# mlakolar/CoordinateDescent.jl

Measured on AMD Instinct MI355X. Metric: coord_updates_per_sec, higher is better.
Workload: dtype f64; 1 GPU; lasso_full_cyclic_sweep_gaussian_n10000000_p1000_f64_allmove; n=10000000, p=1000, s=100, sweep_mode=block32, graph=False, parallelism=rows1

## Files before the change

### coordinatedescent.jl_amd/csrc/cdhip.hip

```cpp
#include "../../include/cdhip.h"

#include <dlfcn.h>
#include <hip/hip_runtime.h>

#include <algorithm>
#include <cmath>
#include <cstdio>
#include <cstdlib>
#include <cstring>
#include <string>
#include <utility>
#include <vector>

#include "kernels.hpp"
#include "gram_kernels.hpp"
#include "vc_kernels.hpp"
#include "vc_gram.hpp"
#include "p2p_exchange.hpp"
#include "sparse_iterate.hpp"
#include "resid_state.hpp"
#include "cache_state.hpp"
#include "exchange_state.hpp"

using namespace cdk;
// ... 281 lines not shown
    int mode = CDH_SWEEP_BLOCK, blockB = 32;
    bool width_default = true, width_agreed = false;
    bool use_graph = false;
    int screening = 1;
    bool reuse_residual = false;
    cdh::ResidState rs;
    bool chunk_dup = false;
    std::vector<int32_t> stamp;
    GraphCache graphs;
    bool graph_broken = false;
    bool domain_error = false;
    int step_grid = 1, block_grid = 1, cus = 1;
    int64_t gram_units = 1;
    Knobs knobs;
    cdh::ExchangeState xs;
    DevBuf<unsigned long long> p2p_inbox;
    cdk::P2PPeers p2p_peers{};
    std::vector<void*> p2p_mapped;
    PinBuf<int> p2p_timeout;
    DevBuf<unsigned> d_p2p_base;
    PinBuf<double> h_xchg;
    size_t h_xchg_doubles = 0;
    GradCache gc;
    CovSolvePath cs;
    SmallPath small;
    bool prof = false;
    double prof_ms = 0.0, prof_bytes = 0.0;
    int64_t prof_launches = 0;
    hipEvent_t ev0 = nullptr, ev1 = nullptr;
    std::string err;
};

#include "quad_solve_types.hpp"
static_assert(kQuadMaxP == CDH_QUAD_MAX_P, "cdhip.h names the limit quad_solve_types.hpp derives");
struct cdh_quad_s {
    int64_t p = 0, max_batch = 0, m = 0;
    int32_t device = 0;
    hipStream_t stream = nullptr;
    unsigned lds_bytes = 0;
    bool A_set = false, penalty_set = false, has_omega = false, omega_shared = false;
    DevBuf<double> A, inv_a, B, omega, lambda0, grid, beta, g, h_out;
    DevBuf<int32_t> sup, nnz, list;
    int64_t list_cap = 0;
    DevBuf<QuadStat> stats;
    PinBuf<QuadStat> h_stats;
    PinBuf<double> h_h;
    std::vector<double> h_B, h_omega, h_lambda0, h_beta;
    std::vector<int32_t> h_sup, h_nnz;
    bool host_stale = true;
};

namespace {

#define HIPCHK(h, call)                                                                     \
    do {                                                                                    \
        hipError_t e_ = (call);                                                             \
        if (e_ != hipSuccess) {                                                             \
            char buf_[512];                                                                 \
            snprintf(buf_, sizeof buf_, "%s failed: %s (%s:%d)", #call, hipGetErrorString(e_), \
                     __FILE__, __LINE__);                                                   \
            (h)->err = buf_;                                                                \
            return e_ == hipErrorOutOfMemory ? CDH_OOM : CDH_HIP_ERROR;                     \
        }                                                                                   \
    } while (0)

#define CHK(call)                                   \
    do {                                            \
        int32_t s_ = (call);                        \
        if (s_ != CDH_OK) return s_;                \
    } while (0)

int32_t fail(cdh_handle h, int32_t code, const char* msg) {
    if (h) h->err = msg; else g_create_error = msg;
    return code;
}

#define NEED_P(h, ptr)                                                         \
    do {                                                                       \
        if (!(ptr)) return fail((h), CDH_BAD_ARG, #ptr " is NULL");            \
    } while (0)

inline int64_t round_up(int64_t a, int64_t b) { return (a + b - 1) / b * b; }

inline int balanced_grid(int64_t units, int64_t gmax) {
    return (int)std::max<int64_t>(1, std::min<int64_t>(gmax, units));
}

template <typename F> int32_t dispatch(cdh_handle h, F&& f) {
    return h->dtype == CDH_F64 ? f((double*)nullptr) : f((float*)nullptr);
}

int32_t upload_ctrl(cdh_handle h) {
    *h->h_ctrl = h->ctrl;
    HIPCHK(h, hipMemcpyAsync(h->d_ctrl, h->h_ctrl, sizeof(Ctrl), hipMemcpyHostToDevice, h->stream));
    return CDH_OK;
}

inline int32_t refused(cdh_handle h, const cdh::Refusal& r) { return r.status == CDH_OK ? (int32_t)CDH_OK : fail(h, r.status, r.msg); }
int32_t exchange_alive(cdh_handle h) { return refused(h, h->xs.alive()); }
int32_t p2p_check(cdh_handle h) {
    if (h->xs.direct_on() && *(volatile int*)h->p2p_timeout) return refused(h, h->xs.p2p_timed_out());
    return CDH_OK;
}

static_assert(GramRec<4>::N <= cdk::kP2PMaxCount, "the widest block record must fit one inbox slot");
cdk::P2PCall next_p2p_call(cdh_handle h) {
    cdh::ExchangeState& xs = h->xs;
    return cdk::P2PCall{h->p2p_peers, xs.rank(), xs.direct_ranks(), xs.next_epoch(), h->knobs.p2p_spin_limit, h->p2p_timeout,
                        xs.in_capture() ? (const unsigned*)h->d_p2p_base : nullptr};
}

int32_t allreduce(cdh_handle h, double* dbuf, size_t count) {
    cdh::ExchangeState& xs = h->xs;
    const cdh::Routing to = xs.route(count);
    switch (to.route) {
    case cdh::Route::Refuse: return refused(h, to.why);
    case cdh::Route::Nothing: return CDH_OK;
    case cdh::Route::Host:
        for (size_t o = 0; o < count; o += h->h_xchg_doubles) {
            const size_t cnt = std::min(h->h_xchg_doubles, count - o);
            HIPCHK(h, hipMemcpyAsync(h->h_xchg, dbuf + o, sizeof(double) * cnt, hipMemcpyDeviceToHost, h->stream));
            HIPCHK(h, hipStreamSynchronize(h->stream));
            const int32_t rc = xs.host_callback()(xs.host_context(), h->h_xchg, (int64_t)cnt);
            if (rc != 0) return fail(h, CDH_RCCL_ERROR, "the host exchange callback reported a failure");
            HIPCHK(h, hipMemcpyAsync(dbuf + o, h->h_xchg, sizeof(double) * cnt, hipMemcpyHostToDevice, h->stream));
            HIPCHK(h, hipStreamSynchronize(h->stream));
        }
        break;
    case cdh::Route::Direct:
        CHK(p2p_check(h));
        for (size_t o = 0; o < count; o += cdk::kP2PMaxCount) {
            const int c = (int)std::min<size_t>(cdk::kP2PMaxCount, count - o);
            hipLaunchKernelGGL(cdk::k_p2p_allreduce, dim3((c + 255) / 256), dim3(256), 0, h->stream, dbuf + o, c,
                               next_p2p_call(h));
            xs.issued(to.route);
        }
        HIPCHK(h, hipGetLastError());
        return CDH_OK;
    case cdh::Route::Rccl: {
        const int rc = g_rccl.AllReduce(dbuf, dbuf, count, kNcclDouble, kNcclSum, xs.communicator(), h->stream);
        if (rc != 0) {
            h->err = std::string("ncclAllReduce failed: ") +
                     (g_rccl.GetErrorString ? g_rccl.GetErrorString(rc) : "?");
            return CDH_RCCL_ERROR;
        }
        break;
    }
    }
    xs.issued(to.route);
    return CDH_OK;
}

int32_t rebuild_residual_from(cdh_handle h, const cdh::SupportList& x, bool with_beta);
int32_t sync_r(cdh_handle h) {
    cdh::ResidState& rs = h->rs;
    if (rs.lazy()) return rebuild_residual_from(h, rs.take_lazy(), false);
    if (rs.pending().empty()) return CDH_OK;
    rs.catchup_begins();
    const cdh::MoveLedger& L = rs.pending();
    for (size_t o = 0; o < L.size(); o += 64) {
        const int cnt = (int)std::min<size_t>(64, L.size() - o);
        for (int i = 0; i < cnt; ++i) { h->h_idx[i] = L[o + (size_t)i]; h->h_hs[i] = L.value(L[o + (size_t)i]); }
        HIPCHK(h, hipMemcpyAsync(h->d_idx, h->h_idx, sizeof(int64_t) * (size_t)cnt, hipMemcpyHostToDevice, h->stream));
        HIPCHK(h, hipMemcpyAsync(h->d_hs, h->h_hs, sizeof(double) * (size_t)cnt, hipMemcpyHostToDevice, h->stream));
        CHK(dispatch(h, [&](auto* t) {
            using T = std::remove_pointer_t<decltype(t)>;
            hipLaunchKernelGGL(k_multi_axpy<T>, dim3(h->step_grid), dim3(kBlock), 0, h->stream, (const T*)h->X, h->ld,
                               h->nvec, (T*)h->r, h->d_idx, h->d_hs, 0, cnt);
            return CDH_OK;
        }));
        HIPCHK(h, hipGetLastError());
        HIPCHK(h, hipStreamSynchronize(h->stream));
        rs.catchup_batch_applied();
    }
    rs.catchup_done();
    h->gc.n_reconcile += 1;
    return CDH_OK;
}

constexpr int64_t kColBatch = 4096;
inline int col_dots_chunks(const cdh_handle_s* h, int64_t bc) {
    const int64_t groups = (bc + kColGroup - 1) / kColGroup;
    const int64_t want_chunks = std::max<int64_t>(1, ((int64_t)h->cus * 8 + groups - 1) / groups);
    return (int)std::max<int64_t>(1, std::min<int64_t>({(int64_t)kColChunks, want_chunks, (h->nvec + kBlock - 1) / kBlock}));
}
int32_t col_dots(cdh_handle h, int64_t j0, int64_t nc, const void* rvec, bool use_w,
                 const int64_t* d_cols = nullptr) {
    if (rvec == h->r) CHK(sync_r(h));
    for (int64_t b0 = 0; b0 < nc; b0 += kColBatch) {
        const int64_t bc = std::min<int64_t>(kColBatch, nc - b0);
        const int64_t groups = (bc + kColGroup - 1) / kColGroup;
        const int chunks = col_dots_chunks(h, bc);
        if ((size_t)groups * chunks * 2 * kColGroup > h->partials_doubles) return fail(h, CDH_BAD_ARG, "partials too small");
        dim3 grid(chunks, (unsigned)groups);
        CHK(dispatch(h, [&](auto* t) {
            using T = std::remove_pointer_t<decltype(t)>;
            hipLaunchKernelGGL(k_col_dots<T>, grid, dim3(kBlock), 0, h->stream, (const T*)h->X, h->ld,
                               h->nvec, use_w ? (const T*)h->w : (const T*)nullptr, (const T*)rvec,
                               j0 + b0, (int)bc, d_cols, h->d_partials);
            return CDH_OK;
        }));
        hipLaunchKernelGGL(k_col_dots_reduce, dim3((unsigned)bc), dim3(64), 0, h->stream,
                           h->d_partials, chunks, h->d_colout + 2 * b0);
        HIPCHK(h, hipGetLastError());
    }
    CHK(allreduce(h, h->d_colout, (size_t)(2 * nc)));
    return CDH_OK;
}

int32_t col_loadings(cdh_handle h) {
    CHK(sync_r(h));
    for (int64_t b0 = 0; b0 < h->p; b0 += kColBatch) {
        const int64_t bc = std::min<int64_t>(kColBatch, h->p - b0);
        const int64_t groups = (bc + kColGroup - 1) / kColGroup;
        const int chunks = col_dots_chunks(h, bc);
        if ((size_t)groups * chunks * kColGroup > h->partials_doubles) return fail(h, CDH_BAD_ARG, "partials too small");
        dim3 grid(chunks, (unsigned)groups);
        CHK(dispatch(h, [&](auto* t) {
            using T = std::remove_pointer_t<decltype(t)>;
            hipLaunchKernelGGL(k_col_loadings<T>, grid, dim3(kBlock), 0, h->stream, (const T*)h->X, h->ld,
                               h->nvec, (const T*)h->r, b0, (int)bc, h->d_partials);
            return CDH_OK;
        }));
        hipLaunchKernelGGL(k_col_loadings_reduce, dim3((unsigned)bc), dim3(64), 0, h->stream,
                           h->d_partials, chunks, h->d_colout + b0);
        HIPCHK(h, hipGetLastError());
    }
    CHK(allreduce(h, h->d_colout, (size_t)h->p));
    return CDH_OK;
}

int32_t resid_moments_dev(cdh_handle h, const void* vec = nullptr, double shift = 0.0, bool sum_w = false) {
    if (!vec) { CHK(sync_r(h)); vec = h->r; }
    const int grid = (int)std::max<int64_t>(1, std::min<int64_t>(1024, (h->nvec + kBlock - 1) / kBlock));
    CHK(dispatch(h, [&](auto* t) {
        using T = std::remove_pointer_t<decltype(t)>;
        auto go = [&](auto kernel) {
            hipLaunchKernelGGL(kernel, dim3(grid), dim3(kBlock), 0, h->stream, h->nvec,
                               (const T*)vec, h->has_w ? (const T*)h->w : (const T*)nullptr, h->d_partials, shift, h->n);
        };
        if (sum_w) go(k_resid_moments<T, true>); else go(k_resid_moments<T>);
        return CDH_OK;
    }));
    hipLaunchKernelGGL(k_sum_records, dim3(1), dim3(kBlock), 0, h->stream, h->d_partials, grid, h->d_red);
    HIPCHK(h, hipGetLastError());
    CHK(allreduce(h, h->d_red, 4));
    return CDH_OK;
}

constexpr int kGcEngage = 3;
constexpr int kGcBusy = 64;
constexpr int kGcMaxFetch = 64;
constexpr int kGcMaxSupport = 512;
constexpr size_t kGcMaxBytes = (size_t)1 << 30;
constexpr int64_t kGcCovWindow = 2048;
constexpr int64_t kGcRowsPerNnz = 400;
constexpr int64_t kGcRowsPerNnzDev = 32;
inline int64_t gc_rows_per_nnz(const cdh_handle_s* h) {
    const GradCache& c = h->gc;
    if (h->knobs.gc_rows_per_nnz > 0) return h->knobs.gc_rows_per_nnz;
    return (c.cov && (c.d_scan || c.g.empty())) ? kGcRowsPerNnzDev : kGcRowsPerNnz;
}

constexpr int kGcMaxSupportShort = 4096;
constexpr size_t kGcShortColumnBytes = (size_t)1 << 20;
inline bool gc_short_columns(const cdh_handle_s* h) {
    return h->gc.cov && (h->gc.d_scan || h->gc.g.empty()) && (size_t)h->n * h->esz <= kGcShortColumnBytes;
}
inline bool gc_support_outgrown(const cdh_handle_s* h) {
    if (h->gc.mode == 3 || gc_short_columns(h)) return false;
    return h->x.nnz() * gc_rows_per_nnz(h) > h->n_total;
}
inline int64_t gc_max_support(const cdh_handle_s* h) { return gc_short_columns(h) ? kGcMaxSupportShort : kGcMaxSupport; }

inline bool gc_applicable(const cdh_handle_s* h) {
    return h->gc.mode != 0 && (h->loss != CDH_WLS || h->has_w);
}
void gc_invalidate(cdh_handle h, bool columns) {
    GradCache& c = h->gc;
    c.st.invalidated(columns);
    if (columns) {
        c.G.clear(); c.G.shrink_to_fit();
        std::fill(c.slot.begin(), c.slot.end(), -1);
        h->cs.colmax_slots = 0;
        c.dev_slots = 0;
        c.full_seen = 0;
    }
}
void gc_after_rebuild(cdh_handle h, const cdh::SupportList& x) { h->gc.st.rebuilt(x, h->p); }
void gc_note_moves(cdh_handle h, const int64_t* idx0, int m) {
    for (int i = 0; i < m; ++i)
        if (h->h_hs[i] != 0.0 && !h->gc.st.moved(idx0[i], h->h_hs[i], cdh::MoveKind::streamed)) return;
}

int32_t upload_beta(cdh_handle h, const cdh::SupportList& x) {
    if (x.nnz() == 0) {
        HIPCHK(h, hipMemsetAsync(h->beta, 0, sizeof(double) * h->p, h->stream));
        return CDH_OK;
    }
    std::vector<double> dense((size_t)h->p, 0.0);
    for (int64_t s = 0; s < x.nnz(); ++s) dense[(size_t)x.coord(s)] = x.slot_value(s);
    HIPCHK(h, hipMemcpyAsync(h->beta, dense.data(), sizeof(double) * h->p, hipMemcpyHostToDevice, h->stream));
    HIPCHK(h, hipStreamSynchronize(h->stream));
    return CDH_OK;
}
int32_t rebuild_residual_from(cdh_handle h, const cdh::SupportList& x, bool with_beta) {
    if (h->rs.rebuild_is_noop(x)) {
        if (with_beta) CHK(upload_beta(h, x));
        h->rs.rebuild_skipped();
        gc_after_rebuild(h, x);
        return CDH_OK;
    }
    h->rs.rebuild_begins();
    if (with_beta) CHK(upload_beta(h, x));
    const int64_t nnz = x.nnz();
    if (nnz == 0) {
        HIPCHK(h, hipMemcpyAsync(h->r, h->y, (size_t)h->ld * h->esz, hipMemcpyDeviceToDevice, h->stream));
    } else {
        std::vector<int64_t> si((size_t)nnz);
        std::vector<double> sv((size_t)nnz);
        for (int64_t s = 0; s < nnz; ++s) { si[(size_t)s] = x.coord(s); sv[(size_t)s] = x.slot_value(s); }
        HIPCHK(h, hipMemcpyAsync(h->d_sup_idx, si.data(), sizeof(int64_t) * nnz, hipMemcpyHostToDevice, h->stream));
        HIPCHK(h, hipMemcpyAsync(h->d_sup_val, sv.data(), sizeof(double) * nnz, hipMemcpyHostToDevice, h->stream));
        const int grid = (int)std::max<int64_t>(1, std::min<int64_t>(2048, (h->nvec + kBlock - 1) / kBlock));
        CHK(dispatch(h, [&](auto* t) {
            using T = std::remove_pointer_t<decltype(t)>;
            hipLaunchKernelGGL(k_init_resid<T>, dim3(grid), dim3(kBlock), 0, h->stream, (const T*)h->X, h->ld,
                               h->nvec, (const T*)h->y, (T*)h->r, h->d_sup_idx, h->d_sup_val, (int)nnz);
            return CDH_OK;
        }));
        HIPCHK(h, hipGetLastError());
        HIPCHK(h, hipStreamSynchronize(h->stream));
    }
    h->rs.rebuilt_from(x);
    gc_after_rebuild(h, x);
    return CDH_OK;
}
int32_t rebuild_residual(cdh_handle h) { return rebuild_residual_from(h, h->x, true); }

void note_duplicates(cdh_handle h, const int64_t* idx0, int m) {
    if ((int64_t)h->stamp.size() != h->p) h->stamp.assign((size_t)h->p, 0);
    h->chunk_dup = false;
    for (int i = 0; i < m; ++i) {
        if (h->stamp[(size_t)idx0[i]]) { h->chunk_dup = true; break; }
        h->stamp[(size_t)idx0[i]] = 1;
    }
    for (int i = 0; i < m; ++i) h->stamp[(size_t)idx0[i]] = 0;
}

int32_t finish_chunk(cdh_handle h, const int64_t* idx0, int m, double* maxH) {
    HIPCHK(h, hipMemcpyAsync(h->h_hs, h->d_hs, sizeof(double) * (size_t)m, hipMemcpyDeviceToHost, h->stream));
    HIPCHK(h, hipMemcpyAsync(h->h_newval, h->d_newval, sizeof(double) * (size_t)m, hipMemcpyDeviceToHost, h->stream));
    HIPCHK(h, hipMemcpyAsync(h->h_touched, h->d_touched, sizeof(int32_t) * (size_t)m, hipMemcpyDeviceToHost, h->stream));
    HIPCHK(h, hipMemcpyAsync(h->h_ctrl, h->d_ctrl, sizeof(Ctrl), hipMemcpyDeviceToHost, h->stream));
    HIPCHK(h, hipStreamSynchronize(h->stream));
    CHK(p2p_check(h));
    if (h->h_ctrl->domain_error) h->domain_error = true;
    const double mh = h->h_ctrl->maxH;
    if (mh > *maxH) *maxH = mh;
    for (int i = 0; i < m; ++i) {
        const int64_t k = idx0[i];
        if (h->h_touched[i] && h->x.get(k) == 0.0) h->x.set(k, 1.0);
        h->x.set(k, h->h_newval[i]);
    }
    gc_note_moves(h, idx0, m);
    return CDH_OK;
}

template <typename T, int B> int32_t launch_block_chunk(cdh_handle h, int m) {
    constexpr int NREC = BlockRec<B>::N;
    const int G = h->block_grid;
    int nprev = 0;
    for (int pos0 = 0; pos0 < m; pos0 += B) {
        const int nb = std::min(B, m - pos0);
        hipLaunchKernelGGL((k_blockstep<T, B>), dim3(G), dim3(kBlock), 0, h->stream, (const T*)h->X,
                           h->ld, h->nvec, (T*)h->r, h->d_idx, h->d_hs, pos0, nb, nprev, h->d_partials);
        if (!h->xs.sharded()) {
            hipLaunchKernelGGL((k_block_finalize<B, true>), dim3(1), dim3(1024), 0, h->stream,
                               h->d_partials, G, nb, h->d_ctrl, h->beta, h->omega, h->d_idx, h->d_hs,
                               h->d_newval, h->d_touched, pos0, h->d_red);
        } else {
            hipLaunchKernelGGL((k_block_finalize<B, false>), dim3(1), dim3(1024), 0, h->stream,
                               h->d_partials, G, nb, h->d_ctrl, h->beta, h->omega, h->d_idx, h->d_hs,
                               h->d_newval, h->d_touched, pos0, h->d_red);
            CHK(allreduce(h, h->d_red, NREC));
            hipLaunchKernelGGL((k_block_scalar<B>), dim3(1), dim3(64), 0, h->stream, h->d_red, nb,
                               h->d_ctrl, h->beta, h->omega, h->d_idx, h->d_hs, h->d_newval,
                               h->d_touched, pos0);
        }
        nprev = nb;
    }
    const int last0 = ((m - 1) / B) * B;
    hipLaunchKernelGGL((k_block_axpy<T, B>), dim3(G), dim3(kBlock), 0, h->stream, (const T*)h->X, h->ld,
                       h->nvec, (T*)h->r, h->d_idx, h->d_hs, last0, m - last0);
    return CDH_OK;
}

constexpr int kGramGridPerCU = 2;
constexpr int kGram32GridPerCU = 3;
constexpr int kLtGridPerCU = 2;
constexpr int gram_blocks_per_cu(int NG, bool lt) {
    return lt ? kLtGridPerCU : NG == 2 ? kGram32GridPerCU : kGramGridPerCU;
}
inline int NGgrid(cdh_handle h, int NG, bool lt = false) {
    return balanced_grid(h->gram_units, (int64_t)h->cus * gram_blocks_per_cu(NG, lt));
}

template <typename T, int NG> int32_t launch_gram_chunk(cdh_handle h, int m) {
    using R = GramRec<NG>;
    constexpr int B = R::B;
    const T* wts = h->has_w ? (const T*)h->w : (const T*)nullptr;
    const int lt = h->knobs.lt;
    const bool use_lt = (lt == 1 || (lt == 2 && (NG >= 2 || h->n >= 2000000))) && !(NG == 4 && sizeof(T) == 4);
    int G = NGgrid(h, NG, use_lt);
    const int64_t rounds64 = ((h->nvec + 63) / 64) / ((int64_t)G * kGramWaves);
    const bool short_chunks = use_lt && (h->knobs.ks == 1 || (h->knobs.ks == 0 && rounds64 < kShortRounds));
    {
        const int64_t cvn = use_lt ? (int64_t)(64 / NG) * (short_chunks ? 1 : NG) : 64;
        const int64_t nchunks = (h->nvec + cvn - 1) / cvn;
        G = balanced_grid((nchunks + kGramWaves - 1) / kGramWaves, (int64_t)h->cus * gram_blocks_per_cu(NG, use_lt));
    }
    if ((size_t)G * R::N > h->partials_doubles) return fail(h, CDH_BAD_ARG, "partial buffer too small for this grid");
    int nprev = 0;
    for (int pos0 = 0; pos0 < m; pos0 += B) {
        const int nb = std::min(B, m - pos0);
        auto go = [&](auto kernel) {
            hipLaunchKernelGGL(kernel, dim3(G), dim3(64 * kGramWaves), 0, h->stream, (const T*)h->X, h->ld, h->nvec,
                               wts, (T*)h->r, h->d_idx, h->d_hs, pos0, nb, nprev, h->d_partials);
        };
        if (use_lt) {
            if constexpr (NG == 1) {
                go(k_gramstep<T, 1, true>);
            } else if constexpr (NG == 4 && sizeof(T) == 4) {
                go(k_gramstep<T, NG>);
            } else {
                if (short_chunks) go(k_gramstep<T, NG, true, 1>); else go(k_gramstep<T, NG, true>);
            }
        } else {
            go(k_gramstep<T, NG>);
        }
        hipLaunchKernelGGL(k_gram_reduce, dim3((R::N + kReduceVals - 1) / kReduceVals), dim3(64 * kReduceWaves), 0, h->stream, h->d_partials, G, R::N, h->d_red);
        CHK(allreduce(h, h->d_red, R::N));
        hipLaunchKernelGGL((k_gram_scalar<NG>), dim3(1), dim3(64), 0, h->stream, h->d_red, nb, h->chunk_dup ? 1 : 0, h->d_ctrl,
                           h->beta, h->omega, h->d_idx, h->d_hs, h->d_newval, h->d_touched, pos0);
        nprev = nb;
    }
    const int last0 = ((m - 1) / B) * B;
    hipLaunchKernelGGL(k_multi_axpy<T>, dim3(h->step_grid), dim3(kBlock), 0, h->stream, (const T*)h->X, h->ld,
                       h->nvec, (T*)h->r, h->d_idx, h->d_hs, last0, m - last0);
    return CDH_OK;
}

template <typename T> int32_t launch_coord_chunk(cdh_handle h, int m) {
    const int G = h->step_grid;
    for (int pos = 0; pos < m; ++pos) {
        if (h->has_w)
            hipLaunchKernelGGL((k_step<T, true>), dim3(G), dim3(kBlock), 0, h->stream, (const T*)h->X,
                               h->ld, h->nvec, (const T*)h->w, (T*)h->r, h->d_idx, h->d_hs, pos, h->d_partials);
        else
            hipLaunchKernelGGL((k_step<T, false>), dim3(G), dim3(kBlock), 0, h->stream, (const T*)h->X,
                               h->ld, h->nvec, (const T*)nullptr, (T*)h->r, h->d_idx, h->d_hs, pos, h->d_partials);
        if (!h->xs.sharded()) {
            hipLaunchKernelGGL(k_finalize<true>, dim3(1), dim3(kBlock), 0, h->stream, h->d_partials, G,
                               h->d_ctrl, h->beta, h->omega, h->d_idx, h->d_hs, h->d_newval, h->d_touched,
                               pos, h->d_red);
        } else {
            hipLaunchKernelGGL(k_finalize<false>, dim3(1), dim3(kBlock), 0, h->stream, h->d_partials, G,
                               h->d_ctrl, h->beta, h->omega, h->d_idx, h->d_hs, h->d_newval, h->d_touched,
                               pos, h->d_red);
            CHK(allreduce(h, h->d_red, 4));
            hipLaunchKernelGGL(k_scalar_update, dim3(1), dim3(64), 0, h->stream, h->d_red, h->d_ctrl,
                               h->beta, h->omega, h->d_idx, h->d_hs, h->d_newval, h->d_touched, pos);
        }
    }
    hipLaunchKernelGGL(k_axpy<T>, dim3(G), dim3(kBlock), 0, h->stream, (const T*)h->X, h->ld, h->nvec,
                       (T*)h->r, h->d_idx, h->d_hs, m);
    return CDH_OK;
}

int32_t all_ranks_agree(cdh_handle h, bool mine, bool* all);
int32_t agree_default_width(cdh_handle h) {
    if (h->width_agreed || !h->width_default || !h->xs.sharded() || h->xs.nranks() <= 1) return CDH_OK;
    bool all64 = false;
    CHK(all_ranks_agree(h, h->blockB == 64, &all64));
    if (!all64) h->blockB = 32;
    h->width_agreed = true;
    return CDH_OK;
}

int32_t run_chunk(cdh_handle h, const int64_t* idx0, int m, double* maxH) {
    CHK(agree_default_width(h));
    CHK(sync_r(h));
    h->rs.stream_begins();
    h->xs.chunk_begins();
    std::memcpy(h->h_idx, idx0, sizeof(int64_t) * (size_t)m);
    note_duplicates(h, idx0, m);
    HIPCHK(h, hipMemcpyAsync(h->d_idx, h->h_idx, sizeof(int64_t) * (size_t)m, hipMemcpyHostToDevice, h->stream));
    h->ctrl.maxH = 0.0;
    h->ctrl.domain_error = 0;
    CHK(upload_ctrl(h));
    if (h->prof) HIPCHK(h, hipEventRecord(h->ev0, h->stream));
    const bool blocked = (h->mode == CDH_SWEEP_BLOCK) && (!h->has_w || h->blockB >= 16);
    auto enqueue = [&]() {
        return dispatch(h, [&](auto* t) {
            using T = std::remove_pointer_t<decltype(t)>;
            if (!blocked) return launch_coord_chunk<T>(h, m);
            if (h->blockB == 64) return launch_gram_chunk<T, 4>(h, m);
            if (h->blockB == 32) return launch_gram_chunk<T, 2>(h, m);
            if (h->blockB == 16) return launch_gram_chunk<T, 1>(h, m);
            if (h->blockB == 8) return launch_block_chunk<T, 8>(h, m);
            if (h->blockB == 4) return launch_block_chunk<T, 4>(h, m);
            return launch_block_chunk<T, 2>(h, m);
        });
    };
    bool launched = false;
    if (h->use_graph && !h->graph_broken && h->xs.may_capture() && m >= (blocked ? 2 * h->blockB : 8)) {
        const uint64_t key = ((uint64_t)m << 20) | ((uint64_t)(blocked ? h->blockB : 0) << 8) | h->xs.graph_key_bits() |
                             (h->chunk_dup ? 4u : 0u) | (h->has_w ? 2u : 0u);
        const GraphEntry* entry = h->graphs.find(key);
        if (!entry) {
            hipGraph_t graph = nullptr;
            hipGraphExec_t exec = nullptr;
            h->xs.capture_begins();
            hipError_t e0 = hipStreamBeginCapture(h->stream, hipStreamCaptureModeThreadLocal);
            const int32_t erc = e0 == hipSuccess ? enqueue() : (int32_t)CDH_HIP_ERROR;
            hipError_t e1 = e0 == hipSuccess ? hipStreamEndCapture(h->stream, &graph) : e0;
            const cdh::Captured holds = h->xs.capture_ends();
            if (erc == CDH_OK && e1 == hipSuccess && graph) e1 = hipGraphInstantiate(&exec, graph, nullptr, nullptr, 0);
            if (graph) (void)hipGraphDestroy(graph);
            if (erc != CDH_OK || e1 != hipSuccess || !exec) {
                (void)hipGetLastError();
                h->graph_broken = true;
            } else {
                entry = h->graphs.insert({key, exec, holds});
            }
        }
        if (entry) {
            if (entry->holds.exchanges)
                hipLaunchKernelGGL(cdk::k_set_u32, dim3(1), dim3(1), 0, h->stream, h->d_p2p_base, h->xs.reserve_epochs(entry->holds.exchanges));
            h->xs.replay_counted(entry->holds);
            HIPCHK(h, hipGraphLaunch(entry->exec, h->stream));
            launched = true;
        }
    }
    if (!launched) CHK(enqueue());
    h->rs.stream_enqueued(blocked ? (m + h->blockB - 1) / h->blockB + 1 : m + 1);
    HIPCHK(h, hipGetLastError());
    if (h->prof) HIPCHK(h, hipEventRecord(h->ev1, h->stream));
    CHK(finish_chunk(h, idx0, m, maxH));
    if (h->prof) {
        float ms = 0.f;
        HIPCHK(h, hipEventElapsedTime(&ms, h->ev0, h->ev1));
        h->prof_ms += ms;
        const double vec = (double)h->n * (double)h->esz;
        if (!blocked) {
            h->prof_launches += m;
            for (int i = 0; i < m; ++i) {
                const bool ap = i > 0 && h->h_hs[i - 1] != 0.0;
                h->prof_bytes += vec * ((h->has_w ? 3.0 : 2.0) + (ap ? 2.0 : 0.0));
            }
            if (h->h_hs[m - 1] != 0.0) h->prof_bytes += 3.0 * vec;
        } else {
            const int B = h->blockB;
            for (int pos0 = 0; pos0 < m; pos0 += B) {
                const int nb = std::min(B, m - pos0);
                int nzp = 0;
                for (int i = std::max(0, pos0 - B); i < pos0; ++i) nzp += h->h_hs[i] != 0.0;
                h->prof_bytes += vec * (nb + 1 + nzp + (nzp ? 1 : 0));
                h->prof_launches += 1;
            }
            int nzl = 0;
            for (int i = ((m - 1) / B) * B; i < m; ++i) nzl += h->h_hs[i] != 0.0;
            if (nzl) h->prof_bytes += vec * (nzl + 2);
        }
    }
    return CDH_OK;
}

constexpr int kScreenMinPass = 16;
#include "grad_cache.hpp"
#include "small_solve.hpp"
#include "cov_solve.hpp"
#include "quad_solve.hpp"
#include "cv_path.hpp"

constexpr int kScreen = 64, kScreenMax = 1024;

int32_t screened_full_pass(cdh_handle h, const int64_t* idx0, int64_t m, double* maxH) {
    {
        bool handled = false;
        CHK(gc_full_pass(h, idx0, m, maxH, &handled));
        if (handled) return CDH_OK;
    }
    const int B = (h->mode == CDH_SWEEP_BLOCK) ? h->blockB : 1;
    GcThresholds T(h, 0.0);
    std::vector<double> cd((size_t)(2 * kScreenMax));
    const int64_t scr_max = std::min<int64_t>({(int64_t)kScreenMax, h->p, h->cap});
    int64_t pos = 0, cool = 0, cool_len = kScreen, scr = std::min<int64_t>(kScreen, scr_max);
    while (pos < m) {
        if (cool > 0) {
            const int mm = (int)std::min<int64_t>({(int64_t)h->cap, m - pos, std::max<int64_t>(cool, B)});
            CHK(run_chunk(h, idx0 + pos, mm, maxH));
            pos += mm; cool -= mm;
            continue;
        }
        const int S = (int)std::min<int64_t>(scr, m - pos);
        std::memcpy(h->h_idx, idx0 + pos, sizeof(int64_t) * (size_t)S);
        HIPCHK(h, hipMemcpyAsync(h->d_idx, h->h_idx, sizeof(int64_t) * (size_t)S, hipMemcpyHostToDevice, h->stream));
        CHK(col_dots(h, 0, S, h->r, h->has_w, h->d_idx));
        HIPCHK(h, hipMemcpyAsync(cd.data(), h->d_colout, sizeof(double) * 2 * S, hipMemcpyDeviceToHost, h->stream));
        if (h->loss == CDH_SQRT) {
            CHK(resid_moments_dev(h));
            HIPCHK(h, hipMemcpyAsync(h->h_red, h->d_red, sizeof(double) * 4, hipMemcpyDeviceToHost, h->stream));
        }
        HIPCHK(h, hipStreamSynchronize(h->stream));
        if (h->loss == CDH_SQRT) T.rnorm = std::sqrt(h->h_red[1]);
        int hit = S;
        for (int i = 0; i < S; ++i) {
            const int64_t k = idx0[pos + i];
            if (h->x.get(k) != 0.0 || !(std::fabs(cd[(size_t)(2 * i)]) <= T.thr_of(k)) || !(cd[(size_t)(2 * i + 1)] > 0.0)) { hit = i; break; }
        }
        for (int i = 0; i < hit; ++i) replay_settled(h, idx0[pos + i], cd[(size_t)(2 * i)] != 0.0);
        pos += hit;
        if (hit < S) {
            const int mm = (int)std::min<int64_t>(std::max(B, 1), m - pos);
            CHK(run_chunk(h, idx0 + pos, mm, maxH));
            pos += mm;
            cool = cool_len; cool_len = std::min<int64_t>(cool_len * 2, m);
            scr = std::min<int64_t>(kScreen, scr_max);
        } else {
            cool_len = kScreen;
            scr = std::min<int64_t>(scr * 2, scr_max);
        }
    }
    return CDH_OK;
}

int32_t run_pass(cdh_handle h, const int64_t* idx0, int64_t m, double* maxH, bool screen = false) {
    *maxH = 0.0;
    if (screen && h->screening && (h->loss != CDH_WLS || h->has_w) && m >= kScreenMinPass && h->x.nnz() * 4 <= h->p) {
        CHK(screened_full_pass(h, idx0, m, maxH));
    } else {
        for (int64_t off = 0; off < m; off += h->cap) {
            const int mm = (int)std::min<int64_t>(h->cap, m - off);
            if (gc_ready_for_cov(h, idx0 + off, mm)) CHK(cov_chunk(h, idx0 + off, mm, maxH));
            else CHK(run_chunk(h, idx0 + off, mm, maxH));
        }
    }
    h->x.dropzeros();
    return CDH_OK;
}

int32_t solve(cdh_handle h, const cdh_options* o, cdh::VisitScheduler& sched, cdh_stats* st) {
    bool prev_converged = false, converged = true;
    std::vector<int64_t> visit;
    st->converged = 0;
    for (int64_t iter = 0; iter < o->maxIter;) {
        {
            int outcome = kCsNotNow;
            CHK(cov_solve(h, o, sched, st, &prev_converged, &converged, &iter, &outcome));
            if (outcome == kCsFinished) break;
            if (outcome == kCsAgain) continue;
        }
        const bool full = converged;
        sched.next_pass(h->x, full, visit);
        double maxH = 0.0;
        if (!visit.empty()) CHK(run_pass(h, visit.data(), (int64_t)visit.size(), &maxH, full));
        else h->x.dropzeros();
        h->gc.st.unprepared();
        st->passes += 1; st->visits += (int64_t)visit.size(); st->maxH = maxH;
        if (full) st->full_passes += 1;
        prev_converged = converged;
        converged = maxH < o->optTol;
        ++iter;
        if (prev_converged && converged) { st->converged = 1; break; }
    }
    st->domain_error = h->domain_error ? 1 : 0;
    return CDH_OK;
}

int32_t lambda_max(cdh_handle h, double* out, std::vector<double>* dots = nullptr ) {
    CHK(col_dots(h, 0, h->p, h->r, h->loss == CDH_WLS));
    std::vector<double> cd_own;
    std::vector<double>& cd = dots ? *dots : cd_own;
    cd.resize((size_t)(2 * h->p));
    HIPCHK(h, hipMemcpyAsync(cd.data(), h->d_colout, sizeof(double) * 2 * h->p, hipMemcpyDeviceToHost, h->stream));
    double denom = (double)h->n_total;
    if (h->loss == CDH_SQRT) {
        CHK(resid_moments_dev(h));
        HIPCHK(h, hipMemcpyAsync(h->h_red, h->d_red, sizeof(double) * 4, hipMemcpyDeviceToHost, h->stream));
    }
    HIPCHK(h, hipStreamSynchronize(h->stream));
    h->rs.dots_taken(cd, h->loss == CDH_WLS);
    if (h->loss == CDH_SQRT) denom = std::sqrt(h->h_red[1]);
    const std::vector<double>& om = h->h_omega;
    double lmax = 0.0;
    for (int64_t k = 0; k < h->p; ++k) {
        double t = std::fabs(-cd[(size_t)(2 * k)] / denom);
        if (h->has_omega) t /= om[(size_t)k];
        if (t > lmax) lmax = t;
    }
    *out = lmax;
    return CDH_OK;
}

void free_all(cdh_handle h) {
    if (!h) return;
    (void)hipSetDevice(h->device);
    if (h->xs.communicator() && g_rccl.CommDestroy) g_rccl.CommDestroy(h->xs.communicator());
    for (void* m : h->p2p_mapped) (void)hipIpcCloseMemHandle(m);
    const hipEvent_t ev[] = {h->ev0, h->ev1};
    const hipStream_t stream = h->stream;
    delete h;
    for (hipEvent_t e : ev) if (e) (void)hipEventDestroy(e);
    if (stream) (void)hipStreamDestroy(stream);
}

template <typename F> int32_t guarded_as(cdh_handle h, F&& body) {
    try { return body(); }
    catch (const std::bad_alloc&) { return fail(h, CDH_OOM, "host allocation failed"); }
    catch (const std::exception& e) { return fail(h, CDH_BAD_ARG, e.what()); }
    catch (...) { return fail(h, CDH_BAD_ARG, "unknown C++ exception"); }
}
template <typename F> int32_t guarded(F&& body) { return guarded_as(nullptr, body); }
template <typename F> int32_t guarded(cdh_handle h, F&& body) {
    if (!h) return fail(nullptr, CDH_BAD_ARG, "handle is NULL");
// ... 1450 lines not shown
```

### coordinatedescent.jl_amd/csrc/gram_kernels.hpp

```cpp
#pragma once
#include <type_traits>

#include "kernels.hpp"

namespace cdk {

typedef double dvec4 __attribute__((ext_vector_type(4)));

template <int NG> struct GramRec {
    static constexpr int B = 16 * NG;
    static constexpr int NT = NG * (NG + 1) / 2;
    static constexpr int OFF_C = NT * 256;
    static constexpr int OFF_Q = OFF_C + B;
    static constexpr int N = OFF_Q + 1;
    __host__ __device__ static constexpr int g(int s, int j) {
        const int gs = s >> 4, gj = j >> 4;
        return tile(gs, gj) * 256 + (s & 15) * 16 + (j & 15);
    }
    __host__ __device__ static constexpr int tile(int gs, int gj) {
        return gs * NG - gs * (gs - 1) / 2 + (gj - gs);
    }
};

constexpr int kGramWaves = 4;
// ... 681 lines not shown
}
struct CovScanOut { int32_t count, nzero, bad_pos, pad; };
__global__ __launch_bounds__(1024) void k_cov_scan(const double* __restrict__ g, const double* __restrict__ a,
                                                   const double* __restrict__ beta, const double* __restrict__ omega,
                                                   const Ctrl* ctrl, const int64_t* __restrict__ idx, int m, int64_t p,
                                                   int32_t* __restrict__ pos_of, uint8_t* __restrict__ setflag,
                                                   int32_t* __restrict__ upos, int64_t* __restrict__ vis,
                                                   double* __restrict__ g_snap, double* __restrict__ beta_snap,
                                                   CovScanOut* out, const uint8_t* __restrict__ forced ) {
    __shared__ int s_wcnt[16];
    __shared__ int s_base, s_nzero;
    const int tid = threadIdx.x, wave = tid >> 6, lane = tid & 63;
    for (int64_t k = tid; k < p; k += 1024) { g_snap[k] = g[k]; beta_snap[k] = beta[k]; pos_of[k] = -1; setflag[k] = 0; }
    if (tid == 0) { s_base = 0; s_nzero = 0; }
    const int loss = ctrl->loss, has_omega = ctrl->has_omega;
    const double thr_base = ctrl->lambda0 * (loss == 1 ? sqrt(ctrl->q_carry) : ctrl->n_total), cert_abs = ctrl->cert_abs;
    __syncthreads();
    for (int i0 = 0; i0 < m; i0 += 1024) {
        const int i = i0 + tid;
        const bool valid = i < m;
        const int64_t k = valid ? idx[i] : 0;
        const double gk = g[k];
        const bool st = valid && forced[k] == 0 && cov_settled(gk, a[k], beta[k], thr_base, has_omega ? omega[k] : 1.0, cert_abs);
        const bool uns = valid && !st;
        if (valid) { pos_of[k] = i; setflag[k] = st ? 1 : 0; }
        if (st && gk == 0.0) atomicAdd(&s_nzero, 1);
        const unsigned long long mask = __ballot(uns);
        if (lane == 0) s_wcnt[wave] = __popcll(mask);
        __syncthreads();
        int before = s_base;
        for (int wv = 0; wv < wave; ++wv) before += s_wcnt[wv];
        if (uns) {
            const int j = before + __popcll(mask & ((1ull << lane) - 1ull));
            upos[j] = i; vis[j] = k;
        }
        __syncthreads();
        if (tid == 0) { int tot = 0; for (int wv = 0; wv < 16; ++wv) tot += s_wcnt[wv]; s_base += tot; }
        __syncthreads();
    }
    if (tid == 0) { out->count = s_base; out->nzero = s_nzero; out->bad_pos = 0x7fffffff; out->pad = 0; }
}
__global__ __launch_bounds__(256) void k_cov_restore(double* __restrict__ g, double* __restrict__ beta,
                                                     const double* __restrict__ g_snap, const double* __restrict__ beta_snap, int64_t p) {
    const int64_t k = (int64_t)blockIdx.x * blockDim.x + threadIdx.x;
    if (k < p) { g[k] = g_snap[k]; beta[k] = beta_snap[k]; }
}
__global__ __launch_bounds__(256) void k_cov_gupdate_chk(double* __restrict__ g, const double* __restrict__ Gcols,
                                                         const int32_t* __restrict__ slot, const double* __restrict__ a,
                                                         const double* __restrict__ omega, const Ctrl* ctrl, int64_t p,
                                                         const int64_t* __restrict__ vis, const double* __restrict__ hs,
                                                         const double* __restrict__ qs, const int32_t* __restrict__ upos,
                                                         const int32_t* __restrict__ pos_of, const uint8_t* __restrict__ setflag,
                                                         int j0, int nb, int m, int last_block, const double* __restrict__ q_start,
                                                         CovScanOut* out, uint8_t* __restrict__ forced) {
    __shared__ double s_h[64], s_q[64];
    __shared__ int64_t s_off[64];
    __shared__ int s_pos[64];
    __shared__ int s_n;
    if (threadIdx.x < 64) {
        const int i = threadIdx.x;
        double h = 0.0, q = 0.0;
        int64_t off = 0;
        int pos = 0;
        if (i < nb) { h = hs[j0 + i]; off = (int64_t)slot[vis[j0 + i]] * p; pos = upos[j0 + i]; q = qs[j0 + i]; }
        const bool nz = (h != 0.0);
        const unsigned long long mask = __ballot(nz);
        if (nz) {
            const int at = __popcll(mask & ((1ull << i) - 1ull));
            s_h[at] = h; s_off[at] = off; s_pos[at] = pos; s_q[at] = q;
        }
        if (i == 0) s_n = __popcll(mask);
    }
    __syncthreads();
    const int nmove = s_n;
    const int64_t k = (int64_t)blockIdx.x * blockDim.x + threadIdx.x;
    if (k >= p) return;
    const int p_prev = j0 > 0 ? upos[j0 - 1] : -1, p_last = last_block ? m - 1 : upos[j0 + nb - 1];
    const int t = pos_of[k];
    bool need = setflag[k] != 0 && t > p_prev && t <= p_last;
    if (nmove == 0 && !need) return;
    const int loss = ctrl->loss;
    double acc = g[k], q_run = *q_start;
    double cert_scale = 0.0, cert_off = 0.0;
    if (need) {
        cert_scale = ctrl->lambda0 * (ctrl->has_omega ? omega[k] : 1.0) * kThrMargin;
        cert_off = ctrl->cert_abs * sqrt(a[k]);
    }
    const double n_total = ctrl->n_total;
    auto holds = [&](double gv, double qv) { return fabs(gv) <= cert_scale * (loss == 1 ? sqrt(qv) : n_total) - cert_off; };
    for (int i = 0; i < nmove; ++i) {
        if (need && s_pos[i] > t) {
            if (!holds(acc, q_run)) { atomicMin(&out->bad_pos, t); forced[k] = 1; }
            need = false;
        }
        acc = fma(-s_h[i], Gcols[s_off[i] + k], acc);
        q_run = s_q[i];
    }
    if (need && !holds(acc, q_run)) { atomicMin(&out->bad_pos, t); forced[k] = 1; }
    if (nmove) g[k] = acc;
}

constexpr int kPackHead = 10;
__global__ __launch_bounds__(256) void k_cov_pack(const Ctrl* ctrl, const CovScanOut* scan, const double* __restrict__ hs,
                                                  const double* __restrict__ newval, const int32_t* __restrict__ touched, int m,
                                                  double* __restrict__ out) {
    const int i = blockIdx.x * blockDim.x + threadIdx.x;
    if (i == 0) {
        *reinterpret_cast<Ctrl*>(out) = *ctrl;
        if (scan) *reinterpret_cast<CovScanOut*>(out + 8) = *scan;
    }
    if (i < m) {
        out[kPackHead + i] = hs[i];
        out[kPackHead + m + i] = newval[i];
        reinterpret_cast<int32_t*>(out + kPackHead + 2 * (size_t)m)[i] = touched[i];
    }
}
static_assert(sizeof(Ctrl) <= 64 && sizeof(CovScanOut) == 16, "k_cov_pack's header layout");

__global__ void k_scatter_f64(double* __restrict__ dst, const int64_t* __restrict__ idx, const double* __restrict__ val, int m) {
    const int i = blockIdx.x * blockDim.x + threadIdx.x;
    if (i < m) dst[idx[i]] = val[i];
}

__global__ __launch_bounds__(256) void k_cov_gupdate(double* __restrict__ g, const double* __restrict__ Gcols,
                                                     const int32_t* __restrict__ slot, int64_t p,
                                                     const int64_t* __restrict__ idx,
                                                     const double* __restrict__ hs, int pos0, int nb) {
    __shared__ double s_h[64];
    __shared__ int64_t s_off[64];
    __shared__ int s_n;
    if (threadIdx.x < 64) {
        const int i = threadIdx.x;
        double h = 0.0;
        int64_t off = 0;
        if (i < nb) { h = hs[pos0 + i]; off = (int64_t)slot[idx[pos0 + i]] * p; }
        const bool nz = (h != 0.0);
        const unsigned long long mask = __ballot(nz);
        if (nz) {
            const int at = __popcll(mask & ((1ull << i) - 1ull));
            s_h[at] = h; s_off[at] = off;
        }
        if (i == 0) s_n = __popcll(mask);
    }
    __syncthreads();
    const int nmove = s_n;
    const int64_t k = (int64_t)blockIdx.x * blockDim.x + threadIdx.x;
    if (k >= p || nmove == 0) return;
    double acc = g[k];
    for (int i = 0; i < nmove; ++i) acc = fma(-s_h[i], Gcols[s_off[i] + k], acc);
    g[k] = acc;
}

template <typename T>
__global__ __launch_bounds__(kBlock) void k_multi_axpy(const T* __restrict__ X, int64_t ld,
                                                       int64_t nvec, T* __restrict__ r,
                                                       const int64_t* __restrict__ idx,
                                                       const double* __restrict__ hs, int pos0,
                                                       int nprev) {
    using V = typename VecOf<T>::V;
    constexpr int NV = VecOf<T>::N;
    __shared__ double s_hp[64];
    __shared__ int64_t s_kp[64];
    __shared__ int s_nzp;
    if (threadIdx.x < 64) {
        const int i = threadIdx.x;
        double h = 0.0;
        int64_t kp = 0;
        if (i < nprev) { h = hs[pos0 + i]; kp = idx[pos0 + i]; }
        const bool nz = (h != 0.0);
        const unsigned long long mask = __ballot(nz);
        if (nz) {
            const int at = __popcll(mask & ((1ull << i) - 1ull));
            s_hp[at] = h; s_kp[at] = kp;
        }
        if (i == 0) s_nzp = __popcll(mask);
    }
    __syncthreads();
    const int nzp = s_nzp;
    if (nzp == 0) return;
    V* __restrict__ rv = reinterpret_cast<V*>(r);
    const int64_t stride = (int64_t)gridDim.x * kBlock;
    for (int64_t j = (int64_t)blockIdx.x * kBlock + threadIdx.x; j < nvec; j += stride) {
        V rr = rv[j];
        double re[NV];
#pragma unroll
        for (int e = 0; e < NV; ++e) re[e] = (double)rr[e];
        for (int i0 = 0; i0 < nzp; i0 += 8) {
            V xp[8];
#pragma unroll
            for (int t = 0; t < 8; ++t) {
                const int ii = (i0 + t < nzp) ? i0 + t : nzp - 1;
                xp[t] = ld_stream<true>(reinterpret_cast<const V*>(X + s_kp[ii] * ld) + j);
            }
#pragma unroll
            for (int t = 0; t < 8; ++t) {
                const double h = (i0 + t < nzp) ? s_hp[i0 + t] : 0.0;
#pragma unroll
                for (int e = 0; e < NV; ++e) re[e] = fma(-h, (double)xp[t][e], re[e]);
            }
        }
#pragma unroll
        for (int e = 0; e < NV; ++e) rr[e] = (T)re[e];
        rv[j] = rr;
    }
}

}
```

### coordinatedescent.jl_amd/csrc/resid_state.hpp

```cpp
#pragma once
#include <cstddef>
#include <cstdint>
#include <vector>

#include "sparse_iterate.hpp"

namespace cdh {

class MoveLedger {
public:
    void resize(int64_t p) {
        val_.assign((std::size_t)p, 0.0); in_.assign((std::size_t)p, 0);
        list_.clear(); list_.reserve((std::size_t)p);
    }
    void add(int64_t k, double d) { join(k); val_[(std::size_t)k] += d; }
    void set(int64_t k, double v) { join(k); val_[(std::size_t)k] = v; }
    double value(int64_t k) const { return val_[(std::size_t)k]; }
    bool contains(int64_t k) const { return in_[(std::size_t)k] != 0; }
    bool empty() const { return list_.empty(); }
    std::size_t size() const { return list_.size(); }
    int64_t operator[](std::size_t i) const { return list_[i]; }
    std::vector<int64_t>::const_iterator begin() const { return list_.begin(); }
    std::vector<int64_t>::const_iterator end() const { return list_.end(); }
    void clear() {
        for (int64_t k : list_) { val_[(std::size_t)k] = 0.0; in_[(std::size_t)k] = 0; }
        list_.clear();
    }

private:
    void join(int64_t k) {
        if (!in_[(std::size_t)k]) { in_[(std::size_t)k] = 1; list_.push_back(k); }
    }
    std::vector<double> val_;
    std::vector<uint8_t> in_;
    std::vector<int64_t> list_;
};

inline bool same_iterate(const SupportList& a, const SupportList& b) {
    if (a.size() != b.size() || a.nnz() != b.nnz()) return false;
    for (int64_t s = 0; s < a.nnz(); ++s) if (a.coord(s) != b.coord(s) || !(a.slot_value(s) == b.slot_value(s))) return false;
    return true;
}

class ResidState {
public:
    void resize(int64_t p) { pending_.resize(p); }

    bool consistent() const { return consistent_; }
    bool lazy() const { return lazy_; }
    const MoveLedger& pending() const { return pending_; }
    bool owes_catchup() const { return lazy_ || !pending_.empty(); }
    int64_t roundings() const { return roundings_; }
    int64_t rebuilds_skipped() const { return n_rebuild_skipped_; }
    int64_t dots_adopted() const { return n_dots_adopted_; }
    bool rebuild_is_noop(const SupportList& x) const {
        return pristine_ && !lazy_ && pending_.empty() && same_iterate(x, x_pristine_);
    }
    bool can_adopt_dots(bool weighted, int64_t p) const {
        return dots_valid_ && dots_w_ == weighted && (int64_t)stash_.size() == 2 * p;
    }

    void stream_begins() { written(); }
    void stream_enqueued(int64_t launches) { roundings_ += launches; }
    void catchup_begins() { pristine_ = false; }
    void catchup_batch_applied() { roundings_ += 1; }
    void catchup_done() { pending_.clear(); }
    const SupportList& take_lazy() { lazy_ = false; return x_lazy_; }
    void rebuild_begins() { overwritten(); roundings_ = 1; }
    void rebuilt_from(const SupportList& x) { consistent_ = true; pristine_ = true; x_pristine_ = x; }
    void rebuild_skipped() { roundings_ = 1; consistent_ = true; n_rebuild_skipped_ += 1; }
    void overwritten_with_y() { consistent_ = false; overwritten(); }
    void regenerated() { overwritten(); }

    void design_or_loss_changed() { consistent_ = false; written(); }
    void iterate_loaded() { consistent_ = false; }
    void iterate_moved() { dots_valid_ = false; }
    void moved(int64_t k, double d) { iterate_moved(); pending_.add(k, d); }
    void left_lazy(const SupportList& x) { dots_valid_ = false; pending_.clear(); lazy_ = true; x_lazy_ = x; consistent_ = true; }

    void dots_taken(const std::vector<double>& cd, bool weighted) { stash_ = cd; dots_valid_ = true; dots_w_ = weighted; }
    void dots_taken(std::vector<double>&& cd, bool weighted) { stash_.swap(cd); dots_valid_ = true; dots_w_ = weighted; }
    const std::vector<double>& adopt_dots() { n_dots_adopted_ += 1; return stash_; }

private:
    void written() { pristine_ = false; dots_valid_ = false; }
    void overwritten() { written(); pending_.clear(); lazy_ = false; }
    bool consistent_ = false, lazy_ = false, pristine_ = false, dots_valid_ = false, dots_w_ = false;
    SupportList x_lazy_, x_pristine_;
    MoveLedger pending_;
    std::vector<double> stash_;
    int64_t roundings_ = 0, n_rebuild_skipped_ = 0, n_dots_adopted_ = 0;
};

}
```

Baseline: 38110 coord-updates/s.

## Defer the final block's residual update until the residual is next needed

```diff
diff --git a/coordinatedescent.jl_amd/csrc/cdhip.hip b/coordinatedescent.jl_amd/csrc/cdhip.hip
--- a/coordinatedescent.jl_amd/csrc/cdhip.hip
+++ b/coordinatedescent.jl_amd/csrc/cdhip.hip
@@ -457,9 +457,26 @@
 }
 
 int32_t rebuild_residual_from(cdh_handle h, const cdh::SupportList& x, bool with_beta);
+static_assert(cdh::kOwedBlockMax == 64, "k_owed_axpy carries 64 moves");
+int32_t pay_owed_block(cdh_handle h) {
+    const std::vector<cdh::OwedMove>& O = h->rs.owed_block();
+    const int cnt = (int)O.size();
+    cdk::OwedBlock blk{};
+    for (int i = 0; i < cnt; ++i) { blk.k[i] = O[(size_t)i].k; blk.h[i] = O[(size_t)i].h; }
+    CHK(dispatch(h, [&](auto* t) {
+        using T = std::remove_pointer_t<decltype(t)>;
+        hipLaunchKernelGGL(k_owed_axpy<T>, dim3(h->step_grid), dim3(kBlock), 0, h->stream, (const T*)h->X, h->ld,
+                           h->nvec, (T*)h->r, blk, cnt);
+        return CDH_OK;
+    }));
+    HIPCHK(h, hipGetLastError());
+    h->rs.owed_block_applied();
+    return CDH_OK;
+}
 int32_t sync_r(cdh_handle h) {
     cdh::ResidState& rs = h->rs;
     if (rs.lazy()) return rebuild_residual_from(h, rs.take_lazy(), false);
+    if (!rs.owed_block().empty()) CHK(pay_owed_block(h));
     if (rs.pending().empty()) return CDH_OK;
     rs.catchup_begins();
     const cdh::MoveLedger& L = rs.pending();
@@ -710,6 +727,9 @@
 inline int NGgrid(cdh_handle h, int NG, bool lt = false) {
     return balanced_grid(h->gram_units, (int64_t)h->cus * gram_blocks_per_cu(NG, lt));
 }
+
+constexpr size_t kOweMinColumnBytes = (size_t)64 << 10;
+inline bool owes_last_block(const cdh_handle_s* h) { return (size_t)h->n * h->esz >= kOweMinColumnBytes; }
 
 template <typename T, int NG> int32_t launch_gram_chunk(cdh_handle h, int m) {
     using R = GramRec<NG>;
@@ -750,6 +770,7 @@
                            h->beta, h->omega, h->d_idx, h->d_hs, h->d_newval, h->d_touched, pos0);
         nprev = nb;
     }
+    if (owes_last_block(h)) return CDH_OK;
     const int last0 = ((m - 1) / B) * B;
     hipLaunchKernelGGL(k_multi_axpy<T>, dim3(h->step_grid), dim3(kBlock), 0, h->stream, (const T*)h->X, h->ld,
                        h->nvec, (T*)h->r, h->d_idx, h->d_hs, last0, m - last0);
@@ -806,6 +827,7 @@
     CHK(upload_ctrl(h));
     if (h->prof) HIPCHK(h, hipEventRecord(h->ev0, h->stream));
     const bool blocked = (h->mode == CDH_SWEEP_BLOCK) && (!h->has_w || h->blockB >= 16);
+    const bool owe = blocked && h->blockB >= 16 && owes_last_block(h);
     auto enqueue = [&]() {
         return dispatch(h, [&](auto* t) {
             using T = std::remove_pointer_t<decltype(t)>;
@@ -849,10 +871,14 @@
         }
     }
     if (!launched) CHK(enqueue());
-    h->rs.stream_enqueued(blocked ? (m + h->blockB - 1) / h->blockB + 1 : m + 1);
+    h->rs.stream_enqueued(blocked ? (m + h->blockB - 1) / h->blockB + (owe ? 0 : 1) : m + 1);
     HIPCHK(h, hipGetLastError());
     if (h->prof) HIPCHK(h, hipEventRecord(h->ev1, h->stream));
     CHK(finish_chunk(h, idx0, m, maxH));
+    if (owe) {
+        const int last0 = ((m - 1) / h->blockB) * h->blockB;
+        h->rs.stream_left_owing(idx0 + last0, h->h_hs + last0, m - last0);
+    }
     if (h->prof) {
         float ms = 0.f;
         HIPCHK(h, hipEventElapsedTime(&ms, h->ev0, h->ev1));
@@ -876,7 +902,7 @@
             }
             int nzl = 0;
             for (int i = ((m - 1) / B) * B; i < m; ++i) nzl += h->h_hs[i] != 0.0;
-            if (nzl) h->prof_bytes += vec * (nzl + 2);
+            if (nzl && !owe) h->prof_bytes += vec * (nzl + 2);
         }
     }
     return CDH_OK;
diff --git a/coordinatedescent.jl_amd/csrc/gram_kernels.hpp b/coordinatedescent.jl_amd/csrc/gram_kernels.hpp
--- a/coordinatedescent.jl_amd/csrc/gram_kernels.hpp
+++ b/coordinatedescent.jl_amd/csrc/gram_kernels.hpp
@@ -857,11 +857,8 @@
 }
 
 template <typename T>
-__global__ __launch_bounds__(kBlock) void k_multi_axpy(const T* __restrict__ X, int64_t ld,
-                                                       int64_t nvec, T* __restrict__ r,
-                                                       const int64_t* __restrict__ idx,
-                                                       const double* __restrict__ hs, int pos0,
-                                                       int nprev) {
+__device__ __forceinline__ void multi_axpy_body(const T* __restrict__ X, int64_t ld, int64_t nvec, T* __restrict__ r,
+                                                const double h, const int64_t kp) {
     using V = typename VecOf<T>::V;
     constexpr int NV = VecOf<T>::N;
     __shared__ double s_hp[64];
@@ -869,9 +866,6 @@
     __shared__ int s_nzp;
     if (threadIdx.x < 64) {
         const int i = threadIdx.x;
-        double h = 0.0;
-        int64_t kp = 0;
-        if (i < nprev) { h = hs[pos0 + i]; kp = idx[pos0 + i]; }
         const bool nz = (h != 0.0);
         const unsigned long long mask = __ballot(nz);
         if (nz) {
@@ -909,5 +903,25 @@
         rv[j] = rr;
     }
 }
-
-}
+template <typename T>
+__global__ __launch_bounds__(kBlock) void k_multi_axpy(const T* __restrict__ X, int64_t ld,
+                                                       int64_t nvec, T* __restrict__ r,
+                                                       const int64_t* __restrict__ idx,
+                                                       const double* __restrict__ hs, int pos0,
+                                                       int nprev) {
+    double h = 0.0;
+    int64_t kp = 0;
+    if (threadIdx.x < 64 && (int)threadIdx.x < nprev) { h = hs[pos0 + threadIdx.x]; kp = idx[pos0 + threadIdx.x]; }
+    multi_axpy_body<T>(X, ld, nvec, r, h, kp);
+}
+struct OwedBlock { int64_t k[64]; double h[64]; };
+template <typename T>
+__global__ __launch_bounds__(kBlock) void k_owed_axpy(const T* __restrict__ X, int64_t ld, int64_t nvec, T* __restrict__ r,
+                                                      const OwedBlock blk, int nprev) {
+    double h = 0.0;
+    int64_t kp = 0;
+    if (threadIdx.x < 64 && (int)threadIdx.x < nprev) { h = blk.h[threadIdx.x]; kp = blk.k[threadIdx.x]; }
+    multi_axpy_body<T>(X, ld, nvec, r, h, kp);
+}
+
+}
diff --git a/coordinatedescent.jl_amd/csrc/resid_state.hpp b/coordinatedescent.jl_amd/csrc/resid_state.hpp
--- a/coordinatedescent.jl_amd/csrc/resid_state.hpp
+++ b/coordinatedescent.jl_amd/csrc/resid_state.hpp
@@ -42,19 +42,23 @@
     return true;
 }
 
+struct OwedMove { int64_t k; double h; };
+constexpr int kOwedBlockMax = 64;
+
 class ResidState {
 public:
-    void resize(int64_t p) { pending_.resize(p); }
+    void resize(int64_t p) { pending_.resize(p); owed_.clear(); owed_.reserve(kOwedBlockMax); }
 
     bool consistent() const { return consistent_; }
     bool lazy() const { return lazy_; }
     const MoveLedger& pending() const { return pending_; }
-    bool owes_catchup() const { return lazy_ || !pending_.empty(); }
+    const std::vector<OwedMove>& owed_block() const { return owed_; }
+    bool owes_catchup() const { return lazy_ || !pending_.empty() || !owed_.empty(); }
     int64_t roundings() const { return roundings_; }
     int64_t rebuilds_skipped() const { return n_rebuild_skipped_; }
     int64_t dots_adopted() const { return n_dots_adopted_; }
     bool rebuild_is_noop(const SupportList& x) const {
-        return pristine_ && !lazy_ && pending_.empty() && same_iterate(x, x_pristine_);
+        return pristine_ && !lazy_ && pending_.empty() && owed_.empty() && same_iterate(x, x_pristine_);
     }
     bool can_adopt_dots(bool weighted, int64_t p) const {
         return dots_valid_ && dots_w_ == weighted && (int64_t)stash_.size() == 2 * p;
@@ -62,6 +66,11 @@
 
     void stream_begins() { written(); }
     void stream_enqueued(int64_t launches) { roundings_ += launches; }
+    void stream_left_owing(const int64_t* idx, const double* hs, int cnt) {
+        owed_.clear();
+        for (int i = 0; i < cnt; ++i) if (hs[i] != 0.0) owed_.push_back({idx[i], hs[i]});
+    }
+    void owed_block_applied() { roundings_ += 1; owed_.clear(); }
     void catchup_begins() { pristine_ = false; }
     void catchup_batch_applied() { roundings_ += 1; }
     void catchup_done() { pending_.clear(); }
@@ -76,7 +85,7 @@
     void iterate_loaded() { consistent_ = false; }
     void iterate_moved() { dots_valid_ = false; }
     void moved(int64_t k, double d) { iterate_moved(); pending_.add(k, d); }
-    void left_lazy(const SupportList& x) { dots_valid_ = false; pending_.clear(); lazy_ = true; x_lazy_ = x; consistent_ = true; }
+    void left_lazy(const SupportList& x) { dots_valid_ = false; pending_.clear(); owed_.clear(); lazy_ = true; x_lazy_ = x; consistent_ = true; }
 
     void dots_taken(const std::vector<double>& cd, bool weighted) { stash_ = cd; dots_valid_ = true; dots_w_ = weighted; }
     void dots_taken(std::vector<double>&& cd, bool weighted) { stash_.swap(cd); dots_valid_ = true; dots_w_ = weighted; }
@@ -84,10 +93,11 @@
 
 private:
     void written() { pristine_ = false; dots_valid_ = false; }
-    void overwritten() { written(); pending_.clear(); lazy_ = false; }
+    void overwritten() { written(); pending_.clear(); owed_.clear(); lazy_ = false; }
     bool consistent_ = false, lazy_ = false, pristine_ = false, dots_valid_ = false, dots_w_ = false;
     SupportList x_lazy_, x_pristine_;
     MoveLedger pending_;
+    std::vector<OwedMove> owed_;
     std::vector<double> stash_;
     int64_t roundings_ = 0, n_rebuild_skipped_ = 0, n_dots_adopted_ = 0;
 };
```

After: 38090 coord-updates/s. No clear change (-0.1%).
